# albertgassol1/vf-nerf

Hardware: AMD Instinct MI355X
Metric: rays/sec (4096-ray chunk, 128 samples/ray) + PSNR vs ref (higher is better)
Workload: dtype f16x3+f32acc

## Files before the change

vf_nerf_amd/csrc/vfn_mlp16.hip:

```cpp
#include <string.h>
#include <utility>
#include "vfn_common.h"
#include "vfn_plan.h"

typedef _Float16 half8 __attribute__((ext_vector_type(8)));
typedef _Float16 half2v __attribute__((ext_vector_type(2)));
typedef float float2v __attribute__((ext_vector_type(2)));
typedef float f32x16 __attribute__((ext_vector_type(16)));
typedef float f32x4v __attribute__((ext_vector_type(4)));

constexpr float VFN16_WSCALE = 64.0f;
constexpr float VFN16_INV_WSCALE = 0.015625f;
constexpr float VFN16_XSCALE = 64.0f;
constexpr int VFN16_SAVE_AUX = 2;
constexpr int VFN16_HANDOVER_NUM = 8;
constexpr int VFN16_DMA_STEPS = 16;
constexpr int VFN16_EPI_PER_MFMA = 6;
constexpr int VFN16_EPI_PER_MFMA2 = 9;
#define VFN16_MAX_CHUNK_KB 39
#define VFN16_STATS_WORDS 64

struct Plan16 {
    int32_t n_hidden;
    int32_t feat_layer;
// ... 137 lines not shown
}

extern "C" int vfn_pack16_weights(int32_t net_kind, const vfn_net_geom* geom, const vfn_layer_params* layers,
                                   void* packed16, void* stream) {
    VfnNetPlan p32; Plan16 p;
    int rc = make_plan16(net_kind, geom, &p32, &p, "vfn_pack16_weights");
    if (rc != VFN_OK) return rc;
    rc = check_kind16(net_kind, p, "vfn_pack16_weights");
    if (rc != VFN_OK) return rc;
    VFN_REQUIRE(layers && packed16, "vfn_pack16_weights: NULL argument");
    Pack16Args a;
    memset(&a, 0, sizeof(a));
    const int L = geom->n_layers, pe_dim = p32.pe_dim, F = geom->feature_dims;
    auto fill = [&](Pack16Entry& e, int i) -> int {
        const vfn_layer_params& q = layers[i];
        VFN_REQUIRE(q.weight && q.bias, "vfn_pack16_weights: layer %d has NULL weight/bias", i);
        e.w = q.weight; e.b = q.bias;
        if (geom->has_bn[i]) {
            VFN_REQUIRE(q.bn_weight && q.bn_bias && q.bn_mean && q.bn_var, "vfn_pack16_weights: layer %d BatchNorm pointer NULL", i);
            e.bn_w = q.bn_weight; e.bn_b = q.bn_bias; e.bn_mean = q.bn_mean; e.bn_var = q.bn_var;
        }
        e.in_dim = geom->in_dims[i]; e.scale = 1.0f;
        return VFN_OK;
    };
    for (int h = 0; h < p.n_hidden; ++h) {
        const int i = p32.hidden[h].ref_layer;
        Pack16Entry& e = a.e[a.n_entries++];
        rc = fill(e, i);
        if (rc != VFN_OK) return rc;
        e.off_kb = p.off_kb[h]; e.n_chunks = p.n_tiles[h]; e.act16 = p.act16[h]; e.aux16 = p.aux16[h];
        const bool feat = p.feat_layer && h == p.n_hidden - 1;
        e.row_off = feat ? 3 : 0;
        e.n_rows = feat ? F : geom->out_dims[i];
        if (net_kind == VFN_NET_VF) {
            if (i == 0) { e.act_valid = 0; e.aux_col_off = 0; e.aux_valid = pe_dim; }
            else if (i == geom->skip_layer) {
                e.act_col_off = 0; e.act_valid = geom->out_dims[i - 1];
                e.aux_col_off = geom->out_dims[i - 1]; e.aux_valid = pe_dim;
                e.scale = 0.70710678118654752440f;
            } else { e.act_col_off = 0; e.act_valid = VFN_HIDDEN; }
        } else {
            if (i == 0) { e.act_col_off = 6 + pe_dim; e.act_valid = F; e.aux_col_off = 0; e.aux_valid = 6 + pe_dim; }
            else { e.act_col_off = 0; e.act_valid = VFN_HIDDEN; }
        }
    }
    {
        Pack16Entry& e = a.e[a.n_entries++];
        rc = fill(e, L - 1);
        if (rc != VFN_OK) return rc;
        e.off_kb = p.head_off_kb; e.n_chunks = 1; e.act16 = 16; e.aux16 = 0;
        e.row_off = 0; e.n_rows = 3; e.act_col_off = 0; e.act_valid = VFN_HIDDEN;
    }
    a.total_words = p.total_kb * 256u;
    a.out = (uint32_t*)packed16;
    a.stats = a.out + a.total_words;
    if (hipMemsetAsync(a.stats, 0, VFN16_STATS_WORDS * 4, (hipStream_t)stream) != hipSuccess) {
        vfn_set_error("vfn_pack16_weights: hipMemsetAsync failed");
        return VFN_ERR_LAUNCH;
    }
    hipLaunchKernelGGL(vfn_pack16_kernel, dim3(a.total_words / 256 + VFN16_STAT_WGS * a.n_entries), dim3(256), 0, (hipStream_t)stream, a);
    return vfn_check_launch("vfn_pack16_weights");
}

namespace {

enum : int { EPI_RELU = 0, EPI_TANH = 1, EPI_HEAD_TANH = 2, EPI_HEAD_SIGMOID = 3 };
enum : int { M16_FEAT = 1, M16_RENDER = 2, M16_TRAIN = 4, M16_BLKOUT = 8, M16_BLKIN = 16, M16_C2 = 32, M16_P1 = 64, M16_SF16 = 128,
             M16_VF_VEC = 0, M16_FUSED = M16_FEAT | M16_RENDER, M16_VF_BLK = M16_FEAT | M16_BLKOUT, M16_RN_BLK = M16_RENDER | M16_BLKIN,
             M16_VF_VEC_TRAIN = M16_TRAIN, M16_VF_FULL_TRAIN = M16_FEAT | M16_TRAIN, M16_FUSED_TRAIN = M16_FUSED | M16_TRAIN };

constexpr int VFN16_FDEPTH = 2;
#define VFN16_SLOT (VFN16_MAX_CHUNK_KB * 64)
#define VFN16_WAVES 4
#define VFN16_PTS 128

typedef __attribute__((address_space(3))) void lds_void;

constexpr int VF_ACT[9] = {0, 16, 16, 16, 14, 16, 16, 16, 16};
constexpr int VF_AUX[9] = {3, 0, 0, 0, 3, 0, 0, 0, 0};
constexpr int VF_TILES[9] = {8, 8, 8, 7, 8, 8, 8, 8, 8};
constexpr int RN_ACT[4] = {16, 16, 16, 16};
constexpr int RN_AUX[4] = {3, 0, 0, 0};
constexpr int RN_TILES[4] = {8, 8, 8, 8};
constexpr int HEAD_KB = 2 * 16 + 1;
constexpr int chunk_kb(int act, int aux) { return 2 * (act + aux) + 1; }
constexpr int vf_off_kb(int h) { int o = 0; for (int i = 0; i < h; ++i) o += VF_TILES[i] * chunk_kb(VF_ACT[i], VF_AUX[i]); return o; }
constexpr int rn_off_kb(int h) { int o = 0; for (int i = 0; i < h; ++i) o += RN_TILES[i] * chunk_kb(RN_ACT[i], RN_AUX[i]); return o; }

struct ChunkD { int net, off_kb, kb, aux; };
constexpr ChunkD chunk_of(int mode, int c) {
    if (!(mode & M16_BLKIN)) {
        const int vf_layers = (mode & M16_FEAT) ? 9 : 8;
        for (int h = 0; h < vf_layers; ++h) {
            if (c < VF_TILES[h]) return {0, vf_off_kb(h) + c * chunk_kb(VF_ACT[h], VF_AUX[h]), chunk_kb(VF_ACT[h], VF_AUX[h]), VF_AUX[h]};
            c -= VF_TILES[h];
        }
        if (c == 0) return {0, vf_off_kb(9), HEAD_KB, 0};
        c -= 1;
    }
    if (mode & M16_RENDER) {
        for (int h = 0; h < 4; ++h) {
            if (c < RN_TILES[h]) return {1, rn_off_kb(h) + c * chunk_kb(RN_ACT[h], RN_AUX[h]), chunk_kb(RN_ACT[h], RN_AUX[h]), RN_AUX[h]};
            c -= RN_TILES[h];
        }
        if (c == 0) return {1, rn_off_kb(4), HEAD_KB, 0};
    }
    return {0, 0, 0, 0};
}

constexpr int rn_first_chunk(int mode) { return (mode & M16_BLKIN) ? 0 : 72; }
constexpr bool chunk_two(int mode, int c) { return (mode & M16_C2) && !(mode & M16_BLKIN) && c >= 63 && c != 71; }
constexpr bool mode_one(int mode) { return (mode & M16_P1) != 0; }
constexpr int VFN16_P1_RING = 5;
#define VFN16_P1_SLOT_KB 20
constexpr int ring_of(int mode) { return mode_one(mode) ? VFN16_P1_RING : 3; }
constexpr int slot_u4(int mode) { return mode_one(mode) ? VFN16_P1_SLOT_KB * 64 : VFN16_MAX_CHUNK_KB * 64; }
constexpr int slot_base(int mode, int c) { return (c % ring_of(mode)) * slot_u4(mode); }
static_assert(VFN16_P1_RING * VFN16_P1_SLOT_KB <= 3 * VFN16_MAX_CHUNK_KB, "the single-product ring must fit into the split modes' ring");
constexpr int stores_of(int mode, int c) { return (c == 0 || ((mode & M16_RENDER) && c == rn_first_chunk(mode))) ? 0 : 4; }
constexpr int young_ops(int mode, int c) {
    const int ring = ring_of(mode);
    int n = 0;
    for (int k = (c - ring + 2 > 0 ? c - ring + 2 : 0); k < c; ++k) n += stores_of(mode, k);
    for (int j = 2; j <= ring - 2; ++j)
        if (c + j >= ring - 1 && chunk_of(mode, c + j).kb > 0) n += (((chunk_of(mode, c + j).kb - 1) / 2 + 1) / VFN16_WAVES);
    return n;
}

struct Mlp16Args {
    const uint4* vf_w;
    const uint4* rn_w;
    const float* points;
    const float* ray_dirs;
    float* out_vec;
    float* out_colors;
    long long n_points;
    int dirs_div;
    int vf_multires, rn_multires;
    uint32_t vf_bytes, rn_bytes;
    float* saved;
    float* save_aux_vf;
    float* save_aux_rn;
    uint32_t* save_masks;
    int save_f16;
    uint4* blk_out;
    const uint4* blk_in;
    const float* vec_in;
    const int* src;
    const int* out_index;
    long long ws_first, ws_points;
    uint32_t* status;
    const int* n_dev;
    unsigned long long* clock;
    long long clock_slots;
};

#define VFN16_CLAMP 60000.0f
constexpr int VFN16_CLAMP_BITS = 0x476a6000;
static_assert(__builtin_bit_cast(int, VFN16_CLAMP) == VFN16_CLAMP_BITS, "VFN16_CLAMP_BITS is VFN16_CLAMP as an integer");

struct X16 { half8 hi[16]; half8 lo[16]; };
struct A16 { half8 hi[3]; half8 lo[3]; };

struct Pipe16 {
    uint4* lds;
    __amdgpu_buffer_rsrc_t vf_w;
// ... 234 lines not shown
                    if ((pr & 3) == 3) {
                        asm volatile("" : "+a"(ehi[sblk]));
                        if constexpr (!P1) asm volatile("" : "+a"(elo[sblk]));
                        if (ch > 0) { xout.hi[2 * (ch > 0 ? ch - 1 : 0) + sblk] = ehi[sblk]; if constexpr (!P1) xout.lo[2 * (ch > 0 ? ch - 1 : 0) + sblk] = elo[sblk]; }
                        else { xpend.hi[PKB + sblk] = ehi[sblk]; if constexpr (!P1) xpend.lo[PKB + sblk] = elo[sblk]; }
                    }
                }
                if constexpr (!P1) {
                __builtin_amdgcn_sched_group_barrier(0x100, W2 ? 1 : 2, 0);
                __builtin_amdgcn_sched_group_barrier(0x008, 1, 0);
                __builtin_amdgcn_sched_group_barrier(0x002, W2 ? VFN16_EPI_PER_MFMA2 : VFN16_EPI_PER_MFMA, 0);
                __builtin_amdgcn_sched_group_barrier(0x008, 1, 0);
                __builtin_amdgcn_sched_group_barrier(0x002, W2 ? VFN16_EPI_PER_MFMA2 : VFN16_EPI_PER_MFMA, 0);
                if (!W2) {
                    __builtin_amdgcn_sched_group_barrier(0x008, 1, 0);
                    __builtin_amdgcn_sched_group_barrier(0x002, VFN16_EPI_PER_MFMA, 0);
                }
                }
            }
            if (st == H - 1 && dnext.kb > 0) {
                if constexpr (P1 && TRAIN) {
                    constexpr int young = young_ops(MODE, C);
                    static_assert(young < 64, "vmcnt is a 6-bit field");
                    if constexpr (young == 0) asm volatile("s_waitcnt vmcnt(0)" ::: "memory");
                    else asm volatile("s_waitcnt vmcnt(%0)" :: "n"(young) : "memory");
                } else
                if (TRAIN && C > 0 && (ch == 0 || ch > 1 || PEPI >= 0)) asm volatile("s_waitcnt vmcnt(4)" ::: "memory");
                else asm volatile("s_waitcnt vmcnt(0)" ::: "memory");
                __builtin_amdgcn_s_barrier();
            }
            if (st >= H && st < H + DST && ddma.kb > 0) {
#pragma unroll
                for (int i = (st - H) * PM / DST; i < (st - H + 1) * PM / DST; ++i) {
                    if (VFN16_WAVES * i + VFN16_WAVES <= DPIECES) dma_piece<ddma.net, ddma.off_kb, slot_base(MODE, C + RING - 1)>(p, piece_blk(wave + VFN16_WAVES * i), lane, P1 ? wave + VFN16_WAVES * i : -1);
                    else if (VFN16_WAVES * i < DPIECES) {
                        const int idx = min(wave + VFN16_WAVES * i, DPIECES - 1);
                        dma_piece<ddma.net, ddma.off_kb, slot_base(MODE, C + RING - 1)>(p, piece_blk(idx), lane, P1 ? idx : -1);
                    }
                }
            }
            if (TRAIN && MPARTS > 0 && st >= H && st < H + MPARTS && (ch > 0 || PEPI >= 0)) {
                static_for<MPARTS>([&](auto ip) {
                    constexpr int part = decltype(ip)::value;
                    if (st - H == part) {
                        if (ch > 0) collect_mask_part<(ch > 0 ? ch - 1 : 0), EPI, part, (MPARTS > 0 ? MPARTS : 1)>(cy, mbits);
                        else collect_mask_part<PKB / 2, (PEPI >= 0 ? PEPI : 0), part, (MPARTS > 0 ? MPARTS : 1)>(cy, mbits);
                    }
                });
            }
            if (TRAIN && st >= DEND && st < DEND + SSTEPS && (ch > 0 || PEPI >= 0)) {
                if (st == DEND) {
                    if constexpr (MPARTS > 0) {
                        if (ch == 0) store_mask<(PSLOT >= 0 ? PSLOT : 0)>(p, cy);
                    } else {
                        if (ch > 0) collect_mask<(ch > 0 ? ch - 1 : 0), EPI>(cy);
                        else { collect_mask<PKB / 2, (PEPI >= 0 ? PEPI : 0)>(cy); store_mask<(PSLOT >= 0 ? PSLOT : 0)>(p, cy); }
                    }
                }
#pragma unroll
                for (int q = (st - DEND) * 4 / SSTEPS; q < (st - DEND + 1) * 4 / SSTEPS; ++q) {
                    if (ch > 0) save_group<(SLOT >= 0 ? SLOT : 0), (ch > 0 ? ch - 1 : 0), (MODE & M16_SF16) != 0>(p, cy.pend, q);
                    else save_group<(PSLOT >= 0 ? PSLOT : 0), PKB / 2, (MODE & M16_SF16) != 0>(p, cy.pend, q);
                }
            }
            if (st == H && ((BLK && ch > 0) || (PBLK && ch == 0))) {
                if (ch > 0) store_blocks<(ch > 0 ? ch - 1 : 0)>(p, xout);
                else store_blocks<PKB / 2>(p, xpend);
            }
            if (st == NKB - 1 && dnext.kb > 0) prefetch_chunk<MODE, (dnext.kb > 0 ? C + 1 : C)>(cy, p, lane);
            __builtin_amdgcn_sched_barrier(0);
        }
        if (EPI == EPI_RELU || EPI == EPI_TANH) {
            cy.pend = acc;
        } else {
#pragma unroll
            for (int c = 0; c < 3; ++c) {
                const float v = acc[c] * VFN16_INV_WSCALE;
                head[c] = (EPI == EPI_HEAD_TANH) ? tanh_exp(v) : 1.0f / (1.0f + expf(-v));
            }
        }
    });
}

__device__ __forceinline__ float enc_value(const float (&x)[3], const float (&sn)[18], const float (&cs)[18], int multires, int k) {
    if (k < 3) return x[k];
    const int idx = k - 3, oct = idx / 6, rem = idx - 6 * oct;
    if (oct >= multires) return 0.f;
    return rem < 3 ? sn[3 * oct + rem] : cs[3 * oct + rem - 3];
}

template <typename F>
__device__ __forceinline__ void build_aux(A16& aux, int g, F col, float& ain) {
#pragma unroll
    for (int s = 0; s < 3; ++s) {
        half8 hi, lo;
#pragma unroll
        for (int j = 0; j < 8; j += 2) {
            float v0, v1;
            if (g == 0) { v0 = col(16 * s + j); v1 = col(16 * s + j + 1); }
            else { v0 = col(16 * s + 8 + j); v1 = col(16 * s + 8 + j + 1); }
            v0 *= VFN16_XSCALE; v1 *= VFN16_XSCALE;
            v0 = fminf(fmaxf(v0, -VFN16_CLAMP), VFN16_CLAMP); v1 = fminf(fmaxf(v1, -VFN16_CLAMP), VFN16_CLAMP);
            ain = fmaxf(ain, fmaxf(fabsf(v0), fabsf(v1)));
            _Float16 h0, h1, l0, l1;
            split2(v0, v1, h0, h1, l0, l1);
            hi[j] = h0; hi[j + 1] = h1; lo[j] = l0; lo[j + 1] = l1;
        }
        aux.hi[s] = hi; aux.lo[s] = lo;
    }
}

template <typename F>
__device__ __forceinline__ void save_aux(float* dst, long long m, int g, F col) {
#pragma unroll
    for (int s = 0; s < 3; ++s)
#pragma unroll
        for (int h = 0; h < 2; ++h) {
            const int c0 = 16 * s + 8 * g + 4 * h;
            if (c0 + 4 <= VFN_AUX_K) {
                f32x4v v;
                if (g == 0) { v = f32x4v{col(16 * s + 4 * h), col(16 * s + 4 * h + 1), col(16 * s + 4 * h + 2), col(16 * s + 4 * h + 3)}; }
                else { v = f32x4v{col(16 * s + 8 + 4 * h), col(16 * s + 8 + 4 * h + 1), col(16 * s + 8 + 4 * h + 2), col(16 * s + 8 + 4 * h + 3)}; }
                *reinterpret_cast<f32x4v*>(dst + m * VFN_AUX_K + c0) = v;
            }
        }
}

__device__ __forceinline__ void load_aux(A16& ax, const float* park) {
    const half8* pk = reinterpret_cast<const half8*>(park + 8);
#pragma unroll
    for (int q = 0; q < 3; ++q) { ax.hi[q] = pk[2 * q]; ax.lo[q] = pk[2 * q + 1]; }
}

__device__ __forceinline__ void encode_sincos(const float (&x)[3], int multires, int g, float (&sn)[18], float (&cs)[18]) {
#pragma unroll
    for (int j = 0; j < 3; ++j)
#pragma unroll
        for (int c = 0; c < 3; ++c) {
            float s = 0.f, k = 0.f;
            if (2 * j < multires) {
                sincosf(x[c] * (g ? (float)(2 << (2 * j)) : (float)(1 << (2 * j))), &s, &k);
                if (2 * j + g >= multires) { s = 0.f; k = 0.f; }
            }
            const float so = __shfl_xor(s, 32, 64), ko = __shfl_xor(k, 32, 64);
            sn[6 * j + c] = g ? so : s;          cs[6 * j + c] = g ? ko : k;
            sn[6 * j + 3 + c] = g ? s : so;      cs[6 * j + 3 + c] = g ? k : ko;
        }
}

template <int MODE>
__device__ __forceinline__ void render_aux(const Mlp16Args& a, A16& aux, const float (&xr)[3], const float (&dr)[3], const float (&nrm)[3],
                                           long long m, bool in, int g, float& ain) {
    const int rn_multires = a.rn_multires;
    float sn[18], cs[18];
    encode_sincos(dr, rn_multires, g, sn, cs);
    const int ncol = 6 + 6 * rn_multires;
    auto rn_col = [&](int k) -> float {
        if (k < 3) return xr[k];
        if (k >= ncol) return k < ncol + 3 ? nrm[k - ncol] : 0.f;
        return enc_value(dr, sn, cs, rn_multires, k - 3);
    };
    build_aux(aux, g, rn_col, ain);
    if ((MODE & M16_TRAIN) && in) save_aux(a.save_aux_rn, m, g, rn_col);
}

template <int MODE>
__device__ __forceinline__ void render_tail(const Mlp16Args& a, const Pipe16& p, Carry16& cy, X16& xa, X16& xb, const A16& aux,
                                            const float (&nrm)[3], long long m, bool in, int wave, int lane) {
    constexpr int R = EPI_RELU, NONE = -1;
    constexpr int C0 = rn_first_chunk(MODE);
    float rgb[3] = {0.f, 0.f, 0.f};
    layer16<MODE, C0 + 0, 16, 3, 8, R, NONE, 0, 9, -1>(xb, aux, xa, xb, cy, rgb, p, wave, lane);
    layer16<MODE, C0 + 8, 16, 0, 8, R, R, 14, 10, 9>(xa, aux, xb, xa, cy, rgb, p, wave, lane);
    layer16<MODE, C0 + 16, 16, 0, 8, R, R, 14, 11, 10>(xb, aux, xa, xb, cy, rgb, p, wave, lane);
    layer16<MODE, C0 + 24, 16, 0, 8, R, R, 14, 12, 11>(xa, aux, xb, xa, cy, rgb, p, wave, lane);
    layer16<MODE, C0 + 32, 16, 0, 1, EPI_HEAD_SIGMOID, R, 14, -1, 12>(xb, aux, xa, xb, cy, rgb, p, wave, lane);
    const long long mo = m;
    if (in && (threadIdx.x & 32) == 0) {
        a.out_vec[mo * 3 + 0] = nrm[0]; a.out_vec[mo * 3 + 1] = nrm[1]; a.out_vec[mo * 3 + 2] = nrm[2];
        a.out_colors[mo * 3 + 0] = rgb[0]; a.out_colors[mo * 3 + 1] = rgb[1]; a.out_colors[mo * 3 + 2] = rgb[2];
    }
}

__device__ __forceinline__ void report_range(const Mlp16Args& a, unsigned long long sat, float ain) {
    if (a.status) {
        const unsigned bits = (sat != 0ull ? 1u : 0u) | (ain >= VFN16_CLAMP ? 2u : 0u);
        if (bits) atomicOr(a.status, bits);
    }
}

template <int MODE>
__global__ __launch_bounds__(256, 1) void vfn_mlp16_kernel(const Mlp16Args a) {
    __shared__ __attribute__((aligned(16))) uint4 s_ring[3 * VFN16_SLOT + 256 * 8];
    float* s_park = reinterpret_cast<float*>(s_ring + 3 * VFN16_SLOT) + threadIdx.x * 32;
    const int tid = threadIdx.x;
    const int lane = tid & 63;
    const int wave = __builtin_amdgcn_readfirstlane(tid >> 6);
    const int g = lane >> 5;
    unsigned long long ck_t0 = 0ull, ck_r0 = 0ull;
    if constexpr ((MODE & M16_RENDER) != 0 && (MODE & M16_BLKIN) == 0 && (MODE & M16_TRAIN) == 0) {
        if (a.clock) { ck_t0 = __builtin_amdgcn_s_memtime(); ck_r0 = __builtin_amdgcn_s_memrealtime(); }
    }
    const long long m = (long long)blockIdx.x * VFN16_PTS + wave * 32 + (lane & 31);
    long long n_live = a.n_points;
    if (a.n_dev) {
        const long long nd = (long long)*a.n_dev;
        n_live = nd < n_live ? nd : n_live;
        if ((long long)blockIdx.x * VFN16_PTS >= n_live) return;
    }
    const bool in = m < n_live;

    if constexpr ((MODE & M16_BLKIN) != 0) {
        const int dpos = in ? a.src[m] : -1;
        const bool live = dpos >= 0;
        float xr[3] = {0.f, 0.f, 0.f}, dr[3] = {0.f, 0.f, 0.f}, nrm[3] = {0.f, 0.f, 0.f};
        if (live) {
            const long long di = dpos / a.dirs_div;
#pragma unroll
            for (int c = 0; c < 3; ++c) { xr[c] = a.points[(long long)dpos * 3 + c]; dr[c] = a.ray_dirs[di * 3 + c]; nrm[c] = a.vec_in[m * 3 + c]; }
        }
        Pipe16 p;
        p.lds = s_ring;
        p.vf_w = __builtin_amdgcn_make_buffer_rsrc(const_cast<uint4*>(a.rn_w), 0, (int)a.rn_bytes, 0x00020000);
        p.rn_w = p.vf_w;
        p.saved = nullptr; p.slot_floats = 0; p.slot_bytes = 0; p.save_voff = 0; p.blk_out = nullptr; p.blk_bytes = 0; p.blk_voff = 0;
        p.masks = nullptr; p.mask_bytes = 0; p.mask_voff = 0; p.save16 = 0; p.save_voff16 = 0; p.feat_voff = 0; p.st_tile = 0; p.st_q = 0;
        dma_chunk<MODE, 0>(p, wave, lane);
        dma_chunk<MODE, 1>(p, wave, lane);
        X16 xa, xb;
        A16 aux;
        float ain_blk = 0.f;
        {
            typedef unsigned int u32x4 __attribute__((ext_vector_type(4)));
            const __amdgpu_buffer_rsrc_t rs_blk = __builtin_amdgcn_make_buffer_rsrc(
                const_cast<uint4*>(a.blk_in), 0, (int)(((a.n_points + 31) & ~31ll) * 1024), 0x00020000);
            const unsigned goff = in ? (unsigned)((m >> 5) * 32768 + lane * 16) : 0xfffffff0u;
            u32x4 q[32];
#pragma unroll
            for (int i = 0; i < 32; ++i) q[i] = __builtin_amdgcn_raw_buffer_load_b128(rs_blk, goff, i * 1024, 0);
            render_aux<MODE>(a, aux, xr, dr, nrm, -1, false, g, ain_blk);
#pragma unroll
            for (int t = 0; t < 8; ++t) {
                half8 h0 = __builtin_bit_cast(half8, q[4 * t + 0]), l0 = __builtin_bit_cast(half8, q[4 * t + 1]);
                half8 h1 = __builtin_bit_cast(half8, q[4 * t + 2]), l1 = __builtin_bit_cast(half8, q[4 * t + 3]);
                asm volatile("" : "+a"(h0)); asm volatile("" : "+a"(l0)); asm volatile("" : "+a"(h1)); asm volatile("" : "+a"(l1));
                xb.hi[2 * t] = h0; xb.lo[2 * t] = l0; xb.hi[2 * t + 1] = h1; xb.lo[2 * t + 1] = l1;
            }
        }
        asm volatile("s_waitcnt vmcnt(0)" ::: "memory");
        __builtin_amdgcn_s_barrier();
        Carry16 cy;
#pragma unroll
        for (int q = 0; q < 16; ++q) cy.pend[q] = 0.f;
        cy.lm[0] = 0; cy.lm[1] = 0; cy.lm[2] = 0; cy.lm[3] = 0; cy.sat = 0ull;
        prefetch_chunk<MODE, 0>(cy, p, lane);
        render_tail<MODE>(a, p, cy, xa, xb, aux, nrm, live ? (long long)dpos : -1, live, wave, lane);
        report_range(a, cy.sat, ain_blk);
    } else {
    float x[3] = {0.f, 0.f, 0.f};
    if (in) { x[0] = a.points[m * 3 + 0]; x[1] = a.points[m * 3 + 1]; x[2] = a.points[m * 3 + 2]; }
    float d[3] = {0.f, 0.f, 0.f};
    int out_row = -1;
    if ((MODE & M16_RENDER) && in) {
        const long long di = m / a.dirs_div;
        d[0] = a.ray_dirs[di * 3 + 0]; d[1] = a.ray_dirs[di * 3 + 1]; d[2] = a.ray_dirs[di * 3 + 2];
        if (a.out_index) out_row = a.out_index[m];
    }
    asm volatile("s_waitcnt vmcnt(0)" ::: "memory");
    if (MODE & M16_RENDER) {
        s_park[0] = x[0]; s_park[1] = x[1]; s_park[2] = x[2];
        s_park[4] = d[0]; s_park[5] = d[1]; s_park[6] = d[2];
    }

    Pipe16 p;
    p.lds = s_ring;
    p.vf_w = __builtin_amdgcn_make_buffer_rsrc(const_cast<uint4*>(a.vf_w), 0, (int)a.vf_bytes, 0x00020000);
    p.rn_w = __builtin_amdgcn_make_buffer_rsrc(const_cast<uint4*>((MODE & M16_RENDER) ? a.rn_w : a.vf_w), 0,
                                               (int)((MODE & M16_RENDER) ? a.rn_bytes : a.vf_bytes), 0x00020000);
    const bool frag = (a.save_f16 & 2) != 0;
    const long long mw = m + a.ws_first;
    p.slot_floats = frag ? ((a.ws_points + 31) >> 5) * 8192 : a.ws_points * 256;
    p.saved = a.saved + a.ws_first * 256;
    {
        const long long left = p.slot_floats * 4 - a.ws_first * 1024;
        p.slot_bytes = (uint32_t)(left < 0x7fffffffll ? left : 0x7fffffffll);
    }
    p.save_voff = !in ? (frag ? 0xc0000000u : 0xfffffff0u) : (frag ? (uint32_t)((m >> 5) * 32768 + lane * 16) : (uint32_t)(m * 1024 + g * 16));
    p.save_voff16 = !in ? (frag ? 0xc0000000u : 0xfffffff0u) : (frag ? (uint32_t)((m >> 5) * 32768 + lane * 8) : (uint32_t)(m * 1024 + g * 8));
    p.feat_voff = in ? (uint32_t)(m * 1024 + g * 16) : 0xfffffff0u;
    p.st_tile = frag ? 4096u : 128u; p.st_q = frag ? 1024u : 32u;
    p.masks = a.save_masks; p.mask_bytes = (uint32_t)(a.ws_points * 32); p.mask_voff = in ? (uint32_t)((2 * mw + g) * 16) : 0xfffffff0u;
    p.save16 = a.save_f16 & 1;
    p.blk_out = a.blk_out; p.blk_bytes = (uint32_t)(((a.n_points + 31) & ~31ll) * 1024);
    p.blk_voff = (uint32_t)((m >> 5) * 32768 + lane * 16);
    dma_chunk<MODE, 0>(p, wave, lane);
    dma_chunk<MODE, 1>(p, wave, lane);
    if constexpr (mode_one(MODE)) static_for<VFN16_P1_RING - 3>([&](auto ic) { dma_chunk<MODE, 2 + decltype(ic)::value>(p, wave, lane); });

    const int vf_multires = a.vf_multires;
    A16 aux;
    float ain = 0.f;
    {
        float sn[18], cs[18];
        encode_sincos(x, vf_multires, g, sn, cs);
        build_aux(aux, g, [&](int k) { return enc_value(x, sn, cs, vf_multires, k); }, ain);
        if ((MODE & M16_TRAIN) && in) save_aux(a.save_aux_vf, mw, g, [&](int k) { return enc_value(x, sn, cs, vf_multires, k); });
        half8* pk = reinterpret_cast<half8*>(s_park + 8);
#pragma unroll
        for (int q = 0; q < 3; ++q) { pk[2 * q] = aux.hi[q]; pk[2 * q + 1] = aux.lo[q]; }
    }
    asm volatile("s_waitcnt vmcnt(0)" ::: "memory");
    __builtin_amdgcn_s_barrier();
    Carry16 cy;
#pragma unroll
    for (int q = 0; q < 16; ++q) cy.pend[q] = 0.f;
    cy.lm[0] = 0; cy.lm[1] = 0; cy.lm[2] = 0; cy.lm[3] = 0; cy.sat = 0ull;
    prefetch_chunk<MODE, 0>(cy, p, lane);

    X16 xa, xb;
    float vec[3] = {0.f, 0.f, 0.f};
    constexpr int R = EPI_RELU, T = EPI_TANH, NONE = -1;
    layer16<MODE, 0, 0, 3, 8, R, NONE, 0, 0, -1>(xa, aux, xb, xb, cy, vec, p, wave, lane);
    layer16<MODE, 8, 16, 0, 8, R, R, 14, 1, 0>(xb, aux, xa, xb, cy, vec, p, wave, lane);
    layer16<MODE, 16, 16, 0, 8, R, R, 14, 2, 1>(xa, aux, xb, xa, cy, vec, p, wave, lane);
    layer16<MODE, 24, 16, 0, 7, R, R, 14, 3, 2>(xb, aux, xa, xb, cy, vec, p, wave, lane);
    { A16 ax; load_aux(ax, s_park); layer16<MODE, 31, 14, 3, 8, R, R, 12, 4, 3>(xa, ax, xb, xa, cy, vec, p, wave, lane); }
    layer16<MODE, 39, 16, 0, 8, R, R, 14, 5, 4>(xb, aux, xa, xb, cy, vec, p, wave, lane);
    layer16<MODE, 47, 16, 0, 8, R, R, 14, 6, 5>(xa, aux, xb, xa, cy, vec, p, wave, lane);
    layer16<MODE, 55, 16, 0, 8, R, R, 14, 7, 6>(xb, aux, xa, xb, cy, vec, p, wave, lane);
    if constexpr (!(MODE & M16_FEAT)) {
        layer16<MODE, 63, 16, 0, 1, EPI_HEAD_TANH, R, 14, -1, 7>(xa, aux, xb, xa, cy, vec, p, wave, lane);
        if (in && g == 0) { a.out_vec[m * 3 + 0] = vec[0]; a.out_vec[m * 3 + 1] = vec[1]; a.out_vec[m * 3 + 2] = vec[2]; }
        report_range(a, cy.sat, ain);
    } else {
    constexpr bool BO = (MODE & M16_BLKOUT) != 0;
    layer16<MODE, 63, 16, 0, 8, T, R, 14, 8, 7, BO, false>(xa, aux, xb, xa, cy, vec, p, wave, lane);
    layer16<MODE, 71, 16, 0, 1, EPI_HEAD_TANH, T, 14, -1, 8, false, BO>(xa, aux, xb, xb, cy, vec, p, wave, lane);
    if constexpr (!(MODE & M16_RENDER)) {
        if (in && g == 0) { a.out_vec[m * 3 + 0] = vec[0]; a.out_vec[m * 3 + 1] = vec[1]; a.out_vec[m * 3 + 2] = vec[2]; }
        report_range(a, cy.sat, ain);
    } else {
    float nrm[3];
#pragma unroll
    for (int c = 0; c < 3; ++c) nrm[c] = __shfl(vec[c], lane & 31, 64);
    const float xr[3] = {s_park[0], s_park[1], s_park[2]};
    const float dr[3] = {s_park[4], s_park[5], s_park[6]};
    A16 raux;
    render_aux<MODE>(a, raux, xr, dr, nrm, (MODE & M16_TRAIN) ? mw : m, in, g, ain);
    render_tail<MODE>(a, p, cy, xa, xb, raux, nrm, a.out_index ? (long long)out_row : m, a.out_index ? out_row >= 0 : in, wave, lane);
    report_range(a, cy.sat, ain);
    if constexpr ((MODE & M16_TRAIN) == 0) {
        if (a.clock && threadIdx.x == 0 && (long long)blockIdx.x < a.clock_slots) {
            const unsigned long long t1 = __builtin_amdgcn_s_memtime(), r1 = __builtin_amdgcn_s_memrealtime();
            a.clock[2 * blockIdx.x] = t1 - ck_t0; a.clock[2 * blockIdx.x + 1] = r1 - ck_r0;
        }
    }
    }
    }
    }
}

int check_vf16(const Plan16& vf, const char* what) {
    bool ok = vf.feat_layer == 1 && vf.n_hidden == 9 && (int)vf.head_off_kb == vf_off_kb(9);
    for (int h = 0; ok && h < 9; ++h)
        ok = vf.act16[h] == VF_ACT[h] && vf.aux16[h] == VF_AUX[h] && vf.n_tiles[h] == VF_TILES[h] && (int)vf.off_kb[h] == vf_off_kb(h);
    if (!ok) { vfn_set_error("%s: the f16x3 kernels are specialised for the shipped vector-field network shape", what); return VFN_ERR_UNSUPPORTED; }
    return VFN_OK;
}
int check_rn16(const Plan16& rn, const char* what) {
    bool ok = rn.n_hidden == 4 && (int)rn.head_off_kb == rn_off_kb(4);
    for (int h = 0; ok && h < 4; ++h)
        ok = rn.act16[h] == RN_ACT[h] && rn.aux16[h] == RN_AUX[h] && rn.n_tiles[h] == RN_TILES[h] && (int)rn.off_kb[h] == rn_off_kb(h);
    if (!ok) { vfn_set_error("%s: the f16x3 kernels are specialised for the shipped rendering network shape", what); return VFN_ERR_UNSUPPORTED; }
    return VFN_OK;
}

}

static int check_kind16(int net_kind, const Plan16& p, const char* what) {
    return net_kind == VFN_NET_VF ? check_vf16(p, what) : check_rn16(p, what);
}

static thread_local uint32_t* t_status_word = nullptr;

uint32_t* vfn_internal_f16x3_status() { return t_status_word; }

extern "C" int vfn_f16x3_set_status(uint32_t* status_word) {
    t_status_word = status_word;
    return VFN_OK;
}

static thread_local unsigned long long* t_clock_probe = nullptr;
static thread_local long long t_clock_slots = 0;

extern "C" int vfn_f16x3_set_clock_probe(uint64_t* stamps, int64_t slots) {
    VFN_REQUIRE(slots >= 0 && (stamps || slots == 0), "vfn_f16x3_set_clock_probe: %lld slots without a buffer", (long long)slots);
    t_clock_probe = reinterpret_cast<unsigned long long*>(stamps);
    t_clock_slots = stamps ? slots : 0;
    return VFN_OK;
}

VfnReportScope::VfnReportScope(uint32_t* status_word, uint64_t* clock_stamps, int64_t clock_slots)
    : old_status(t_status_word), old_clock(t_clock_probe), old_slots(t_clock_slots) {
    if (status_word) t_status_word = status_word;
    if (clock_stamps && clock_slots > 0) { t_clock_probe = reinterpret_cast<unsigned long long*>(clock_stamps); t_clock_slots = clock_slots; }
}
VfnReportScope::~VfnReportScope() { t_status_word = old_status; t_clock_probe = old_clock; t_clock_slots = old_slots; }

extern "C" int vfn_vf_mlp16_fwd(const vfn_net_geom* geom, const void* packed16, const float* points, int64_t n_points,
                                 float* out_vec, void* stream) {
    Mlp16Args a = {};
    VfnNetPlan p32; Plan16 vf;
    int rc = make_plan16(VFN_NET_VF, geom, &p32, &vf, "vfn_vf_mlp16_fwd");
    if (rc != VFN_OK) return rc;
    rc = check_vf16(vf, "vfn_vf_mlp16_fwd");
    if (rc != VFN_OK) return rc;
    if (n_points <= 0) return VFN_OK;
    VFN_REQUIRE(packed16 && points && out_vec, "vfn_vf_mlp16_fwd: NULL argument");
    a.vf_w = (const uint4*)packed16; a.points = points; a.out_vec = out_vec; a.n_points = n_points; a.dirs_div = 1;
    a.vf_multires = vf.multires; a.vf_bytes = vf.total_kb * 1024u;
    a.status = t_status_word;
    a.clock = t_clock_probe; a.clock_slots = t_clock_slots;
    const long long blocks = (n_points + VFN16_PTS - 1) / VFN16_PTS;
    hipLaunchKernelGGL(vfn_mlp16_kernel<M16_VF_VEC>, dim3((unsigned)blocks), dim3(256), 0, (hipStream_t)stream, a);
    return vfn_check_launch("vfn_vf_mlp16_fwd");
}

static int launch_fused16(const char* what, const vfn_net_geom* vf_geom, const void* vf_packed16, const vfn_net_geom* rn_geom,
                          const void* rn_packed16, const float* points, const float* ray_dirs, int64_t n_points,
                          int32_t samples_per_ray, const int32_t* out_index, bool scatter, int32_t colour_products, float* normals,
                          float* colors, void* stream, const int32_t* n_dev = nullptr) {
    Mlp16Args a = {};
    a.n_dev = n_dev;
    VfnNetPlan p32; Plan16 vf, rn;
    VFN_REQUIRE(vf_geom && rn_geom, "%s: NULL argument", what);
    int rc = make_plan16(VFN_NET_VF, vf_geom, &p32, &vf, what);
    if (rc != VFN_OK) return rc;
    rc = make_plan16(VFN_NET_RENDER, rn_geom, &p32, &rn, what);
    if (rc != VFN_OK) return rc;
    rc = check_vf16(vf, what);
    if (rc != VFN_OK) return rc;
    rc = check_rn16(rn, what);
    if (rc != VFN_OK) return rc;
    VFN_REQUIRE(vf_geom->feature_dims == VFN_HIDDEN && rn_geom->feature_dims == VFN_HIDDEN, "%s: both nets need feature_dims == %d", what, VFN_HIDDEN);
    VFN_REQUIRE(colour_products == 2 || colour_products == 3, "%s: colour_products must be 2 or 3 (got %d)", what, colour_products);
    if (n_points <= 0) return VFN_OK;
    VFN_REQUIRE(vf_packed16 && rn_packed16 && points && ray_dirs && normals && colors && (out_index || !scatter), "%s: NULL argument", what);
    VFN_REQUIRE(samples_per_ray > 0, "%s: samples_per_ray must be > 0", what);
    a.vf_w = (const uint4*)vf_packed16; a.rn_w = (const uint4*)rn_packed16; a.points = points; a.ray_dirs = ray_dirs;
    a.out_vec = normals; a.out_colors = colors; a.out_index = out_index; a.n_points = n_points; a.dirs_div = samples_per_ray;
    a.vf_multires = vf.multires; a.rn_multires = rn.multires; a.vf_bytes = vf.total_kb * 1024u; a.rn_bytes = rn.total_kb * 1024u;
    a.status = t_status_word;
    a.clock = t_clock_probe; a.clock_slots = t_clock_slots;
// ... 181 lines not shown
```

Baseline: 2.062 million.

## Share per-ray view-direction sincos across wave lanes and fix multires at compile time

The positional-encoding frequency counts become compile-time constants checked against the plan. The render path then detects when a wave covers at most five rays. In that case each lane computes one sincos of a per-ray direction component and octave, and the 24 encoded values are gathered with ds_bpermute instead of every sample recomputing sincos. This removes redundant transcendental work for samples that share a ray, at the cost of extra cross-lane reductions, permutes and an LDS park slot.

```diff
diff --git a/vf_nerf_amd/csrc/vfn_mlp16.hip b/vf_nerf_amd/csrc/vfn_mlp16.hip
--- a/vf_nerf_amd/csrc/vfn_mlp16.hip
+++ b/vf_nerf_amd/csrc/vfn_mlp16.hip
@@ -243,6 +243,9 @@
 constexpr int RN_ACT[4] = {16, 16, 16, 16};
 constexpr int RN_AUX[4] = {3, 0, 0, 0};
 constexpr int RN_TILES[4] = {8, 8, 8, 8};
+constexpr int VF_MULTIRES = 6;
+constexpr int RN_MULTIRES = 4;
+static_assert(VF_MULTIRES % 2 == 0 && RN_MULTIRES % 2 == 0, "encode_sincos pairs the octaves up between the two lane halves");
 constexpr int HEAD_KB = 2 * 16 + 1;
 constexpr int chunk_kb(int act, int aux) { return 2 * (act + aux) + 1; }
 constexpr int vf_off_kb(int h) { int o = 0; for (int i = 0; i < h; ++i) o += VF_TILES[i] * chunk_kb(VF_ACT[i], VF_AUX[i]); return o; }
@@ -643,24 +646,30 @@
     });
 }
 
-__device__ __forceinline__ float enc_value(const float (&x)[3], const float (&sn)[18], const float (&cs)[18], int multires, int k) {
+template <int L>
+__device__ __forceinline__ float enc_value(const float (&x)[3], const float (&sn)[3 * L], const float (&cs)[3 * L], int k) {
     if (k < 3) return x[k];
     const int idx = k - 3, oct = idx / 6, rem = idx - 6 * oct;
-    if (oct >= multires) return 0.f;
+    if (oct >= L) return 0.f;
     return rem < 3 ? sn[3 * oct + rem] : cs[3 * oct + rem - 3];
 }
 
 template <typename F>
-__device__ __forceinline__ void build_aux(A16& aux, int g, F col, float& ain) {
+__device__ __forceinline__ void half_cols(float (&v)[24], int g, F col) {
+#pragma unroll
+    for (int i = 0; i < 24; ++i) {
+        const int k = 16 * (i >> 3) + (i & 7);
+        v[i] = g ? col(k + 8) : col(k);
+    }
+}
+
+__device__ __forceinline__ void build_aux(A16& aux, const float (&v)[24], float& ain) {
 #pragma unroll
     for (int s = 0; s < 3; ++s) {
         half8 hi, lo;
 #pragma unroll
         for (int j = 0; j < 8; j += 2) {
-            float v0, v1;
-            if (g == 0) { v0 = col(16 * s + j); v1 = col(16 * s + j + 1); }
-            else { v0 = col(16 * s + 8 + j); v1 = col(16 * s + 8 + j + 1); }
-            v0 *= VFN16_XSCALE; v1 *= VFN16_XSCALE;
+            float v0 = v[8 * s + j] * VFN16_XSCALE, v1 = v[8 * s + j + 1] * VFN16_XSCALE;
             v0 = fminf(fmaxf(v0, -VFN16_CLAMP), VFN16_CLAMP); v1 = fminf(fmaxf(v1, -VFN16_CLAMP), VFN16_CLAMP);
             ain = fmaxf(ain, fmaxf(fabsf(v0), fabsf(v1)));
             _Float16 h0, h1, l0, l1;
@@ -671,19 +680,14 @@
     }
 }
 
-template <typename F>
-__device__ __forceinline__ void save_aux(float* dst, long long m, int g, F col) {
+__device__ __forceinline__ void save_aux(float* dst, long long m, int g, const float (&v)[24]) {
 #pragma unroll
     for (int s = 0; s < 3; ++s)
 #pragma unroll
         for (int h = 0; h < 2; ++h) {
             const int c0 = 16 * s + 8 * g + 4 * h;
-            if (c0 + 4 <= VFN_AUX_K) {
-                f32x4v v;
-                if (g == 0) { v = f32x4v{col(16 * s + 4 * h), col(16 * s + 4 * h + 1), col(16 * s + 4 * h + 2), col(16 * s + 4 * h + 3)}; }
-                else { v = f32x4v{col(16 * s + 8 + 4 * h), col(16 * s + 8 + 4 * h + 1), col(16 * s + 8 + 4 * h + 2), col(16 * s + 8 + 4 * h + 3)}; }
-                *reinterpret_cast<f32x4v*>(dst + m * VFN_AUX_K + c0) = v;
-            }
+            if (c0 + 4 <= VFN_AUX_K)
+                *reinterpret_cast<f32x4v*>(dst + m * VFN_AUX_K + c0) = f32x4v{v[8 * s + 4 * h], v[8 * s + 4 * h + 1], v[8 * s + 4 * h + 2], v[8 * s + 4 * h + 3]};
         }
 }
 
@@ -693,36 +697,67 @@
     for (int q = 0; q < 3; ++q) { ax.hi[q] = pk[2 * q]; ax.lo[q] = pk[2 * q + 1]; }
 }
 
-__device__ __forceinline__ void encode_sincos(const float (&x)[3], int multires, int g, float (&sn)[18], float (&cs)[18]) {
-#pragma unroll
-    for (int j = 0; j < 3; ++j)
+template <int L>
+__device__ __forceinline__ void encode_sincos(const float (&x)[3], int g, float (&sn)[3 * L], float (&cs)[3 * L]) {
+#pragma unroll
+    for (int j = 0; j < L / 2; ++j)
 #pragma unroll
         for (int c = 0; c < 3; ++c) {
-            float s = 0.f, k = 0.f;
-            if (2 * j < multires) {
-                sincosf(x[c] * (g ? (float)(2 << (2 * j)) : (float)(1 << (2 * j))), &s, &k);
-                if (2 * j + g >= multires) { s = 0.f; k = 0.f; }
-            }
+            float s, k;
+            sincosf(x[c] * (g ? (float)(2 << (2 * j)) : (float)(1 << (2 * j))), &s, &k);
             const float so = __shfl_xor(s, 32, 64), ko = __shfl_xor(k, 32, 64);
             sn[6 * j + c] = g ? so : s;          cs[6 * j + c] = g ? ko : k;
             sn[6 * j + 3 + c] = g ? s : so;      cs[6 * j + 3 + c] = g ? k : ko;
         }
 }
 
+constexpr int VFN16_SHARE_RAYS = 5;
+constexpr int VFN16_SHARE_IDLE = 4 * 12 * VFN16_SHARE_RAYS;
+static_assert(12 * VFN16_SHARE_RAYS + 1 <= 64 && RN_MULTIRES == 4, "12 items per ray and one idle lane in a wave of 64");
+
+__device__ __forceinline__ void view_share(const float* __restrict__ ray_dirs, long long r_min, long long r_max, bool any, long long ray,
+                                           bool live, int lane, int& code, float& arg) {
+    code = -1; arg = 0.f;
+    if (any && r_max - r_min < VFN16_SHARE_RAYS) {
+        const int q = lane / 12, item = lane - 12 * q, o = item / 3, c = item - 3 * o;
+        float comp = 0.f;
+        if (r_min + q <= r_max) comp = ray_dirs[(r_min + q) * 3 + c];
+        arg = comp * (float)(1 << o);
+        code = live ? 48 * (int)(ray - r_min) : VFN16_SHARE_IDLE;
+    }
+}
+
+__device__ __forceinline__ int wave_uniform(int v) { return __builtin_amdgcn_readfirstlane(v); }
+__device__ __forceinline__ long long wave_uniform(long long v) {
+    return (long long)(((unsigned long long)(unsigned)__builtin_amdgcn_readfirstlane((int)(v >> 32)) << 32) | (unsigned)__builtin_amdgcn_readfirstlane((int)v));
+}
+
 template <int MODE>
 __device__ __forceinline__ void render_aux(const Mlp16Args& a, A16& aux, const float (&xr)[3], const float (&dr)[3], const float (&nrm)[3],
-                                           long long m, bool in, int g, float& ain) {
-    const int rn_multires = a.rn_multires;
-    float sn[18], cs[18];
-    encode_sincos(dr, rn_multires, g, sn, cs);
-    const int ncol = 6 + 6 * rn_multires;
-    auto rn_col = [&](int k) -> float {
+                                           long long m, bool in, int g, float& ain, int code, float arg) {
+    constexpr int L = RN_MULTIRES;
+    float sn[3 * L], cs[3 * L];
+    if (wave_uniform(code) >= 0) {
+        float s, k;
+        sincosf(arg, &s, &k);
+#pragma unroll
+        for (int i = 0; i < 3 * L; ++i) {
+            const int from = code == VFN16_SHARE_IDLE ? VFN16_SHARE_IDLE : code + 4 * i;
+            sn[i] = __builtin_bit_cast(float, __builtin_amdgcn_ds_bpermute(from, __builtin_bit_cast(int, s)));
+            cs[i] = __builtin_bit_cast(float, __builtin_amdgcn_ds_bpermute(from, __builtin_bit_cast(int, k)));
+        }
+    } else {
+        encode_sincos<L>(dr, g, sn, cs);
+    }
+    constexpr int ncol = 6 + 6 * L;
+    float v[24];
+    half_cols(v, g, [&](int k) -> float {
         if (k < 3) return xr[k];
         if (k >= ncol) return k < ncol + 3 ? nrm[k - ncol] : 0.f;
-        return enc_value(dr, sn, cs, rn_multires, k - 3);
-    };
-    build_aux(aux, g, rn_col, ain);
-    if ((MODE & M16_TRAIN) && in) save_aux(a.save_aux_rn, m, g, rn_col);
+        return enc_value<L>(dr, sn, cs, k - 3);
+    });
+    build_aux(aux, v, ain);
+    if ((MODE & M16_TRAIN) && in) save_aux(a.save_aux_rn, m, g, v);
 }
 
 template <int MODE>
@@ -775,10 +810,18 @@
         const int dpos = in ? a.src[m] : -1;
         const bool live = dpos >= 0;
         float xr[3] = {0.f, 0.f, 0.f}, dr[3] = {0.f, 0.f, 0.f}, nrm[3] = {0.f, 0.f, 0.f};
+        const int di = live ? dpos / a.dirs_div : -1;
         if (live) {
-            const long long di = dpos / a.dirs_div;
-#pragma unroll
-            for (int c = 0; c < 3; ++c) { xr[c] = a.points[(long long)dpos * 3 + c]; dr[c] = a.ray_dirs[di * 3 + c]; nrm[c] = a.vec_in[m * 3 + c]; }
+#pragma unroll
+            for (int c = 0; c < 3; ++c) { xr[c] = a.points[(long long)dpos * 3 + c]; dr[c] = a.ray_dirs[(long long)di * 3 + c]; nrm[c] = a.vec_in[m * 3 + c]; }
+        }
+        int sh_code; float sh_arg;
+        {
+            int lo = live ? di : 0x7fffffff, hi = di;
+#pragma unroll
+            for (int o = 32; o > 0; o >>= 1) { lo = min(lo, __shfl_xor(lo, o, 64)); hi = max(hi, __shfl_xor(hi, o, 64)); }
+            lo = wave_uniform(lo); hi = wave_uniform(hi);
+            view_share(a.ray_dirs, lo, hi, hi >= 0, di, live, lane, sh_code, sh_arg);
         }
         Pipe16 p;
         p.lds = s_ring;
@@ -799,7 +842,7 @@
             u32x4 q[32];
 #pragma unroll
             for (int i = 0; i < 32; ++i) q[i] = __builtin_amdgcn_raw_buffer_load_b128(rs_blk, goff, i * 1024, 0);
-            render_aux<MODE>(a, aux, xr, dr, nrm, -1, false, g, ain_blk);
+            render_aux<MODE>(a, aux, xr, dr, nrm, -1, false, g, ain_blk, sh_code, sh_arg);
 #pragma unroll
             for (int t = 0; t < 8; ++t) {
                 half8 h0 = __builtin_bit_cast(half8, q[4 * t + 0]), l0 = __builtin_bit_cast(half8, q[4 * t + 1]);
@@ -822,15 +865,24 @@
     if (in) { x[0] = a.points[m * 3 + 0]; x[1] = a.points[m * 3 + 1]; x[2] = a.points[m * 3 + 2]; }
     float d[3] = {0.f, 0.f, 0.f};
     int out_row = -1;
-    if ((MODE & M16_RENDER) && in) {
-        const long long di = m / a.dirs_div;
-        d[0] = a.ray_dirs[di * 3 + 0]; d[1] = a.ray_dirs[di * 3 + 1]; d[2] = a.ray_dirs[di * 3 + 2];
-        if (a.out_index) out_row = a.out_index[m];
+    int sh_code = -1;
+    float sh_arg = 0.f;
+    if constexpr ((MODE & M16_RENDER) != 0) {
+        const long long di = in ? m / a.dirs_div : 0;
+        if (in) {
+            d[0] = a.ray_dirs[di * 3 + 0]; d[1] = a.ray_dirs[di * 3 + 1]; d[2] = a.ray_dirs[di * 3 + 2];
+            if (a.out_index) out_row = a.out_index[m];
+        }
+        const long long left = n_live - ((long long)blockIdx.x * VFN16_PTS + wave * 32);
+        const int last = left > 31 ? 31 : left > 0 ? (int)left - 1 : 0;
+        const long long r_max = (long long)(((unsigned long long)(unsigned)__builtin_amdgcn_readlane((int)(di >> 32), last) << 32) |
+                                            (unsigned)__builtin_amdgcn_readlane((int)di, last));
+        view_share(a.ray_dirs, wave_uniform(di), r_max, left > 0, di, in, lane, sh_code, sh_arg);
     }
     asm volatile("s_waitcnt vmcnt(0)" ::: "memory");
     if (MODE & M16_RENDER) {
-        s_park[0] = x[0]; s_park[1] = x[1]; s_park[2] = x[2];
-        s_park[4] = d[0]; s_park[5] = d[1]; s_park[6] = d[2];
+        s_park[0] = x[0]; s_park[1] = x[1]; s_park[2] = x[2]; s_park[3] = __builtin_bit_cast(float, sh_code);
+        s_park[4] = d[0]; s_park[5] = d[1]; s_park[6] = d[2]; s_park[7] = sh_arg;
     }
 
     Pipe16 p;
@@ -858,14 +910,14 @@
     dma_chunk<MODE, 1>(p, wave, lane);
     if constexpr (mode_one(MODE)) static_for<VFN16_P1_RING - 3>([&](auto ic) { dma_chunk<MODE, 2 + decltype(ic)::value>(p, wave, lane); });
 
-    const int vf_multires = a.vf_multires;
     A16 aux;
     float ain = 0.f;
     {
-        float sn[18], cs[18];
-        encode_sincos(x, vf_multires, g, sn, cs);
-        build_aux(aux, g, [&](int k) { return enc_value(x, sn, cs, vf_multires, k); }, ain);
-        if ((MODE & M16_TRAIN) && in) save_aux(a.save_aux_vf, mw, g, [&](int k) { return enc_value(x, sn, cs, vf_multires, k); });
+        float sn[3 * VF_MULTIRES], cs[3 * VF_MULTIRES], v[24];
+        encode_sincos<VF_MULTIRES>(x, g, sn, cs);
+        half_cols(v, g, [&](int k) { return enc_value<VF_MULTIRES>(x, sn, cs, k); });
+        build_aux(aux, v, ain);
+        if ((MODE & M16_TRAIN) && in) save_aux(a.save_aux_vf, mw, g, v);
         half8* pk = reinterpret_cast<half8*>(s_park + 8);
 #pragma unroll
         for (int q = 0; q < 3; ++q) { pk[2 * q] = aux.hi[q]; pk[2 * q + 1] = aux.lo[q]; }
@@ -907,7 +959,7 @@
     const float xr[3] = {s_park[0], s_park[1], s_park[2]};
     const float dr[3] = {s_park[4], s_park[5], s_park[6]};
     A16 raux;
-    render_aux<MODE>(a, raux, xr, dr, nrm, (MODE & M16_TRAIN) ? mw : m, in, g, ain);
+    render_aux<MODE>(a, raux, xr, dr, nrm, (MODE & M16_TRAIN) ? mw : m, in, g, ain, __builtin_bit_cast(int, s_park[3]), s_park[7]);
     render_tail<MODE>(a, p, cy, xa, xb, raux, nrm, a.out_index ? (long long)out_row : m, a.out_index ? out_row >= 0 : in, wave, lane);
     report_range(a, cy.sat, ain);
     if constexpr ((MODE & M16_TRAIN) == 0) {
@@ -922,14 +974,14 @@
 }
 
 int check_vf16(const Plan16& vf, const char* what) {
-    bool ok = vf.feat_layer == 1 && vf.n_hidden == 9 && (int)vf.head_off_kb == vf_off_kb(9);
+    bool ok = vf.feat_layer == 1 && vf.n_hidden == 9 && (int)vf.head_off_kb == vf_off_kb(9) && vf.multires == VF_MULTIRES;
     for (int h = 0; ok && h < 9; ++h)
         ok = vf.act16[h] == VF_ACT[h] && vf.aux16[h] == VF_AUX[h] && vf.n_tiles[h] == VF_TILES[h] && (int)vf.off_kb[h] == vf_off_kb(h);
     if (!ok) { vfn_set_error("%s: the f16x3 kernels are specialised for the shipped vector-field network shape", what); return VFN_ERR_UNSUPPORTED; }
     return VFN_OK;
 }
 int check_rn16(const Plan16& rn, const char* what) {
-    bool ok = rn.n_hidden == 4 && (int)rn.head_off_kb == rn_off_kb(4);
+    bool ok = rn.n_hidden == 4 && (int)rn.head_off_kb == rn_off_kb(4) && rn.multires == RN_MULTIRES;
     for (int h = 0; ok && h < 4; ++h)
         ok = rn.act16[h] == RN_ACT[h] && rn.aux16[h] == RN_AUX[h] && rn.n_tiles[h] == RN_TILES[h] && (int)rn.off_kb[h] == rn_off_kb(h);
     if (!ok) { vfn_set_error("%s: the f16x3 kernels are specialised for the shipped rendering network shape", what); return VFN_ERR_UNSUPPORTED; }
```

Result: no change. 2.080 million (median of 6 runs) (+0.9%).
